# M4THYOU/TokenDagger

Hardware: AMD Instinct MI355X
Metric: GB/s raw text tokenized (Llama-4 vocab, 1024 MB corpus) (higher is better)
Workload: dtype u8; 1 GPU; Llama-4-Scout vocab, 1024 MiB synthetic english text, 1741775 documents, CoreBPE::encode semantics, input resident in HBM; bytes=1073741824, docs=1741775, bytes_rank0=1073741824, docs_rank0=1741775, parallelism=single GPU

## Files before the change

### tokendagger_amd/csrc/td_common.h

```cpp
#pragma once
#include <stdint.h>

#include "../../include/tokendagger_hip.h"

#if defined(__HIP__)
#define TD_HD __host__ __device__ inline __attribute__((always_inline))
#else
#define TD_HD inline
#endif

namespace td {

enum : uint32_t {
    C_OTHER = 0,
    C_APOS = 1,
    C_SLASH = 2,
    C_SP = 3,
    C_WS = 4,
    C_CRLF = 5,
    C_UP = 6,
    C_LW = 7,
    C_LB = 8,
    C_MK = 9,
    C_NUM = 10,
// ... 721 lines not shown
    }
    TD_HD int run_end2(int k1, int k2, int from) const {
        int i = from;
        while (i < lim) {
            const int wi = i >> 6, sh = i & 63;
            const uint64_t m = ((word(k1, wi) | word(k2, wi)) & ~eword(wi)) >> sh;
            const int t = td_ctz64(~m);
            if (t < 64 - sh) return i + t;
            i += 64 - sh;
        }
        return i;
    }
    template <class F>
    TD_HD int last_where(const F& f, int lo, int hi) const {
        if (hi <= lo) return -1;
        for (int wi = (hi - 1) >> 6; wi >= (lo >> 6); --wi) {
            uint64_t m = f(wi);
            const int base = wi << 6;
            if (hi - base < 64) m &= td_bits_below(hi - base);
            if (lo > base) m &= ~td_bits_below(lo - base);
            if (m) return base + td_top64(m) - 1;
        }
        return -1;
    }
    TD_HD int last_and(int k1, int k2, int lo, int hi) const {
        return last_where([&](int wi) { return word(k1, wi) & word(k2, wi); }, lo, hi);
    }
    TD_HD int last_set(int k, int lo, int hi) const {
        return last_where([&](int wi) { return word(k, wi); }, lo, hi);
    }
    TD_HD int last_clear(int k, int lo, int hi) const {
        return last_where([&](int wi) { return ~word(k, wi); }, lo, hi);
    }
};

template <class P, class B>
TD_HD int scan_contraction_p(const P& p, const B& bytes, int e, bool leading = false) {
    if (e + 3 > p.lim) return -1;
    if (!p.bit(MK_A, e) || (p.bit(MK_D, e) && !leading)) return e;
    if (p.bit(MK_D, e + 1)) return e;
    const uint32_t b1 = bytes(e + 1);
    const bool d2 = p.bit(MK_D, e + 2);
    if (b1 < 0x80) {
        const uint32_t l1 = b1 | 0x20;
        if (l1 == 's' || l1 == 't' || l1 == 'm' || l1 == 'd') return e + 2;
        if (d2) return e;
        const uint32_t b2 = bytes(e + 2);
        if (b2 < 0x80) {
            const uint32_t l2 = b2 | 0x20;
            if ((l1 == 'r' && l2 == 'e') || (l1 == 'v' && l2 == 'e') || (l1 == 'l' && l2 == 'l')) return e + 3;
        }
        return e;
    }
    if (b1 == 0xC5 && !d2 && bytes(e + 2) == 0xBF) return e + 3;
    return e;
}

template <class P, class B>
TD_HD int scan_piece_gpt2_p(const P& p, const B& bytes) {
    const int o = p.o, lim = p.lim;
    if (o + 3 > lim) return -1;
    if (p.bit(MK_A, o) && !p.bit(MK_D, o + 1)) {
        const uint32_t b1 = bytes(o + 1);
        if (b1 == 's' || b1 == 't' || b1 == 'm' || b1 == 'd') return o + 2;
        if (!p.bit(MK_D, o + 2)) {
            const uint32_t b2 = bytes(o + 2);
// ... 306 lines not shown
```

### tokendagger_amd/csrc/td_kernels.hip

```cpp
#include <hip/hip_runtime.h>
#include <stdlib.h>

#include "td_kernels.h"

namespace td {

#ifdef TD_ABLATE
#define TD_STOP(n) (a.stop_after == (n))
#else
#define TD_STOP(n) false
#endif

struct LdsSrc {
    const uint8_t* txt;
    const uint32_t* docw;
    int64_t lo, hi;
    __device__ __forceinline__ uint32_t byte(int64_t i) const { return txt[i]; }
    __device__ __forceinline__ bool doc(int64_t i) const { return (docw[i >> 5] >> (i & 31)) & 1u; }
};
struct GlobSrc {
    const uint8_t* text;
    const uint32_t* docbits;
    int64_t lo, hi;
    __device__ __forceinline__ uint32_t byte(int64_t i) const { return text[i]; }
// ... 220 lines not shown
            const bool less = lo + lane < hi && a.doc_offsets[lo + lane] < b0;
            lo += (int64_t)__popcll((unsigned long long)__ballot(less));
        }
        wave_sync_lds();
        for (int64_t d = lo + lane;; d += 64) {
            const int64_t p = d < nd ? a.doc_offsets[d] : b1;
            if (p >= b0 && p < b1 && p < a.n) {
                atomicOr(&bits[(p - b0) >> 5], 1u << (p & 31));
                atomicMin(&first[(p - b0) / K_TILE], (uint32_t)d);
            }
            if (!((__ballot(p < b1 && d < nd) >> 63) & 1ull)) break;
        }
        wave_sync_lds();
#pragma unroll
        for (int q = 0; q < 4; ++q) {
            const int64_t gw = (b0 >> 5) + 4 * (lane + 64 * q);
            if (gw < words) reinterpret_cast<uint4*>(a.docbits)[gw >> 2] = reinterpret_cast<const uint4*>(bits)[lane + 64 * q];
        }
        const int64_t t = b0 / K_TILE + lane;
        if (lane < PM_RANGE / K_TILE && t <= a.n_tiles) a.tile_first_doc[t] = first[lane];
        wave_sync_lds();
    }
}

constexpr int K_MWORDS = K_WIN / 64;

__device__ __forceinline__ uint64_t bits64(const uint32_t* arr, int pos) {
    const int w = pos >> 5, sh = pos & 31;
    const uint64_t lo = ((uint64_t)arr[w + 1] << 32) | arr[w];
    const uint64_t hi = arr[w + 2];
    return sh ? (lo >> sh) | (hi << (64 - sh)) : lo;
}

template <uint32_t PV>
__device__ __noinline__ int scan_piece_lds(const uint64_t* s_mask, const uint8_t* s_txt, int p) {
    const ArrMaskP mp(s_mask, p, K_LIM);
    return scan_piece_p(mp, [s_txt](int q) { return (uint32_t)s_txt[q]; }, PV);
}

__device__ __forceinline__ void load_bitwin(BitWin& w, const uint64_t* s_mask, int base) {
    const int word = base >> 6, sh = base & 63;
    const uint64_t* lo = s_mask + word * MK_COUNT;
    const uint64_t* hi = lo + MK_COUNT;
#pragma unroll
    for (int k = 0; k < MK_COUNT; ++k) w.m[k] = sh ? (lo[k] >> sh) | (hi[k] << (64 - sh)) : lo[k];
}

__device__ __noinline__ uint4 load_text16_edge(const uint8_t* text, int64_t n, int64_t g) {
    uint32_t w[4] = {0, 0, 0, 0};
    for (int k = 0; k < 16; ++k) {
        const int64_t gg = g + k;
        if (gg >= 0 && gg < n) w[k >> 2] |= (uint32_t)text[gg] << ((k & 3) * 8);
    }
    return make_uint4(w[0], w[1], w[2], w[3]);
}
__device__ __forceinline__ uint4 load_text16(const EncodeArgs& a, int64_t g) {
    if (g >= 0 && g + 16 <= a.n && a.text_aligned) return *reinterpret_cast<const uint4*>(a.text + g);
    if (g + 16 > 0 && g < a.n) return load_text16_edge(a.text, a.n, g);
    return make_uint4(0, 0, 0, 0);
}

__device__ __noinline__ uint32_t stage_window_edge(uint8_t* s_txt, const uint8_t* text, int64_t n, int64_t w0, int tid, int n16) {
    uint32_t hib = 0;
    for (int v = tid; v < n16; v += K_THREADS) {
        const int64_t g = w0 + (int64_t)v * 16;
        uint32_t w[4] = {0, 0, 0, 0};
        for (int k = 0; k < 16; ++k) {
            const int64_t gg = g + k;
            if (gg >= 0 && gg < n) w[k >> 2] |= (uint32_t)text[gg] << ((k & 3) * 8);
// ... 242 lines not shown
        int mine = -1;
        const uint32_t o = k + fz_shift_of(meta, pnm, k, &mine);
        if ((v & 0xC0000000u) == TOK_MISS && mine >= 0) {
            const uint32_t nq = meta[mine] >> 16;
            for (uint32_t q = 0; q < nq; ++q) dst[o + q] = (int32_t)mids[mine * 64 + q];
        } else {
            dst[o] = (int32_t)v;
        }
    }
}
__device__ __forceinline__ void fz_stage_with_misses(const uint32_t* slab, uint32_t* st0, uint32_t* mo0, uint32_t pnp, uint32_t pn0, uint32_t pnm) {
    const uint32_t* const meta = slab + SLAB_META;
    const uint32_t* const mids = slab + SLAB_MIDS;
    for (uint32_t k = threadIdx.x; k < pnp; k += K_THREADS) {
        uint32_t v = slab[k];
        if ((v & 0xC0000000u) == TOK_MISS) {
            for (uint32_t q = 0; q < pnm; ++q) {
                const uint32_t e = meta[q];
                if ((e & 0xFFFFu) == k) {
                    const uint32_t mp = meta[SLAB_MAX_MISSES + q], hq = mp >> 12, pos = mp & 0xFFFu, nq = e >> 16;
                    uint32_t* const mo = mo0 + (size_t)hq * K_STAGE + pos;
                    for (uint32_t r = 0; r < nq; ++r) mo[r] = mids[q * 64 + r];
                    v = TOK_MISS | TOK_MERGED | (pos << 7) | nq;
                }
            }
        }
        if (k < pn0) st0[k] = v; else st0[K_STAGE + (k - pn0)] = v;
    }
}

#ifndef TD_SPLIT_MIN_WAVES
#define TD_SPLIT_MIN_WAVES 6
#endif
constexpr int KS_HCAP = 768;
constexpr int KS_CCAP = 128;

constexpr int FZ_NPC = 5120;
#ifndef TD_FZ_PB
#define TD_FZ_PB 1
#endif
constexpr int FZ_PB = TD_FZ_PB;
constexpr int FZ_R_MASK = (K_MWORDS + 1) * MK_COUNT * 8;
constexpr int FZ_R_HEADS = FZ_R_MASK;
constexpr int FZ_R_COLD = FZ_R_HEADS + (KS_HCAP + 2) * 2;
constexpr int FZ_R_SPLIT_END = FZ_R_COLD + KS_CCAP * 2;
constexpr int FZ_R_PLIST = 0;
constexpr int FZ_CCAP = 768;
constexpr int FZ_R_COLDK = ((FZ_NPC + 8) * 2 + 15) & ~15;
constexpr int FZ_R_PB = FZ_R_COLDK + FZ_CCAP * 2;
constexpr int FZ_R_SM = FZ_R_PB + K_THREADS * 2;
constexpr int FZ_R_TOK_END = FZ_R_SM + K_THREADS * 4;
static_assert(SLAB_MIDS >= FZ_NPC + 8, "a slab holds the slots of the fullest tile the fused loop takes");
constexpr int FZ_R_BYTES = ((FZ_R_SPLIT_END > FZ_R_TOK_END ? FZ_R_SPLIT_END : FZ_R_TOK_END) + 15) & ~15;
constexpr int PD_KIND = 0;
constexpr int PD_TILE = 1, PD_NP = 2, PD_N0 = 3, PD_COUNT = 4, PD_NMISS = 5, PD_FDD = 6, PD_EXT0 = 7;
constexpr int PD_WORDS = 8;
static_assert(SLAB_MAX_MISSES == 2 * K_MISS_LISTED_MAX, "slab layout");
#ifndef TD_LB_MAX_POLLS
#define TD_LB_MAX_POLLS 2
#endif
#ifndef TD_LB_DRAIN_POLLS
#define TD_LB_DRAIN_POLLS 64
#endif
#ifndef TD_LB_MAX_ROUNDS
#define TD_LB_MAX_ROUNDS 4
#endif
#ifndef TD_FUSED_MIN_WAVES
#define TD_FUSED_MIN_WAVES 6
#endif

template <uint32_t PV, bool FUSED, bool DIRECT>
__global__ __launch_bounds__(K_THREADS, FUSED ? TD_FUSED_MIN_WAVES : TD_SPLIT_MIN_WAVES) void td_split_tiles(const EncodeArgs a_kern) {
    static_assert(FUSED || !DIRECT, "direct placement is part of the fused tile loop");
    __shared__ __attribute__((aligned(16))) uint8_t s_txt[K_WIN];
    __shared__ __attribute__((aligned(16))) uint8_t s_R[FZ_R_BYTES];
    uint64_t* const s_mask = reinterpret_cast<uint64_t*>(s_R);
    uint16_t* const s_heads = reinterpret_cast<uint16_t*>(s_R + FZ_R_HEADS);
    uint16_t* const s_cold = reinterpret_cast<uint16_t*>(s_R + FZ_R_COLD);
    __shared__ uint32_t s_start[K_WIN / 32 + 3];
    __shared__ uint32_t s_doc[K_WIN / 32 + 2];
    __shared__ uint8_t s_lut[128];
    __shared__ uint8_t s_fcls[16];
    __shared__ uint32_t s_nh, s_cur, s_ncold, s_nonascii;
    __shared__ int s_last;
    __shared__ int s_cross;
    __shared__ uint32_t s_defer;
    __shared__ int s_next[2];

    const int tid = threadIdx.x;
#ifdef TD_FUSED_TIMING
    unsigned long long tt[16] = {0, 0, 0, 0, 0, 0, 0, 0, 0, 0, 0, 0, 0, 0, 0, 0}, t_last = __builtin_readcyclecounter(), t_total0 = t_last, n_tiles_done = 0;
#define FZ_TICK(i) { const unsigned long long t_now = __builtin_readcyclecounter(); tt[i] += t_now - t_last; t_last = t_now; FZ_FRESH }
#else
#define FZ_TICK(i) FZ_FRESH
#endif
#ifndef TD_ARGS_IN_REGISTERS
    (void)a_kern;
    FreshArgs a{kernarg_args()};
    FreshTables T{(const __attribute__((address_space(4))) Tables*)a->Tp};
#define FZ_FRESH { a.refresh(); T.refresh(); }
#else
    const KeptArgs a{&a_kern};
    const Tables T_kept = uniform_tables(a->Tp);
    const KeptTables T{&T_kept};
#define FZ_FRESH
#endif
    for (int q = tid; q < 128; q += K_THREADS) s_lut[q] = (uint8_t)feature_of_class(T->ascii_cls[q]);
    if (tid < 16) s_fcls[tid] = (uint8_t)feature_of_class((uint32_t)tid);
    if (tid == 0) s_nonascii = 0;
    __shared__ __attribute__((aligned(16))) uint32_t s_kmask[FUSED ? (P12_MAXLEN + 1) * 4 : 4];
    __shared__ uint32_t s_wave[8];
    __shared__ uint32_t s_hflags[2], s_nrec[2], s_ncoldp;
    __shared__ uint32_t s_rec[2][K_MISS_LISTED_MAX];
    __shared__ unsigned long long s_pend[48];
    __shared__ uint32_t s_npend;
    __shared__ uint32_t s_flagl[32];
    __shared__ uint32_t s_nflagl;
    __shared__ uint32_t s_pd[DIRECT ? SLAB_RING : 1][PD_WORDS];
    __shared__ uint32_t s_stat[2];
    __shared__ unsigned long long s_lbv[4];
    __shared__ uint32_t s_lbs[4][3];
    __shared__ uint32_t s_brk;
    auto append_pending = [&](uint32_t npd) {
        const int ln = tid & 63;
        const bool have = (uint32_t)ln < npd;
        const unsigned long long rec = have ? s_pend[ln] : 0ull;
        const uint32_t c = mq_class((uint32_t)rec & 127u);
#pragma unroll
        for (uint32_t q = 0; q < (uint32_t)K_MISS_CLASSES; ++q) {
            const uint64_t b = __ballot(have && c == q);
            if (b) {
                const int leader = (int)td_ctz64(b);
                uint32_t at = 0;
                if (ln == leader) at = atomicAdd(&a->miss_count[q], (uint32_t)__popcll((unsigned long long)b));
                at = (uint32_t)__shfl((int)at, leader);
                if (have && c == q) a->miss_list[(size_t)q * a->miss_cap + at + (uint32_t)__popcll((unsigned long long)(b & ((1ull << ln) - 1ull)))] = rec;
            }
        }
    };
    if constexpr (FUSED) {
        if (tid < (int)(P12_MAXLEN + 1) * 4) {
            const int len = tid >> 2, w = tid & 3, nb = len - 4 * w;
// ... 251 lines not shown
                    uint32_t m0 = 0, m1 = 0;
                    for (uint32_t q = 0; q < pnm; ++q) { if (meta[SLAB_MAX_MISSES + q] >> 12) m1 = 1; else m0 = 1; }
                    a->tile_count[tB4] = pn0 | (m0 ? TILE_MISS_LISTED : 0u);
                    a->tile_extra[tB4] = pext0;
                    if (ptwo) {
                        a->tile_count[tB4 + 1] = (pnp - pn0) | (m1 ? TILE_MISS_LISTED : 0u);
                        a->tile_extra[tB4 + 1] = pcount - pnp - pext0;
                    }
                    if (base == -1) {
                        __hip_atomic_store(&a->tile_state[B], TS_BROKEN << 62, __ATOMIC_RELAXED, __HIP_MEMORY_SCOPE_AGENT);
                        s_brk = 1u;
                    } else {
                        s_stat[1] += 1u;
                    }
                }
            }
            if (tid == 0) s_pd[ring][PD_KIND] = 0;
            FZ_TICK(11)
        }
        if (!have) {
            __syncthreads();
            ring = __builtin_amdgcn_readfirstlane(ring + 1 == SLAB_RING ? 0 : ring + 1);
            continue;
        }
        {
        FZ_TICK(0)
        const bool tile_ascii = !s_nonascii;

        LdsSrc src;
        src.txt = s_txt;
        src.docw = s_doc;
        src.lo = (wg0 < 0) ? -wg0 : 0;
        src.hi = (a->n - wg0 < K_WIN) ? (a->n - wg0) : K_WIN;
        if (tid < MK_COUNT) s_mask[K_MWORDS * MK_COUNT + tid] = 0;
        auto emit_masks = [&](int it, uint32_t flo, uint32_t fhi, uint32_t pf) {
            const uint64_t P = transpose8x8(((uint64_t)fhi << 32) | flo);
            const uint32_t plo = (uint32_t)P, phi = (uint32_t)(P >> 32);
            const uint32_t mU = plo & 0xFF, mW = (plo >> 8) & 0xFF, mX = (plo >> 16) & 0xFF, mS = plo >> 24;
            const uint32_t nraw = phi & 0xFF, mCR = (phi >> 8) & 0xFF, mSL = (phi >> 16) & 0xFF, mC = phi >> 24;
            const uint32_t mN = nraw & ~mX & ~mS, mA = nraw & mX, mSP = nraw & mS;
            const uint32_t mD = reinterpret_cast<const uint8_t*>(s_doc)[it];
            const uint32_t mSY = sync_byte(mU, mW, mX, mS, mN, mCR, mSL, mC, mD, mA, pf, PV);
            static_assert(MK_U == 0 && MK_W == 1 && MK_X == 2 && MK_S == 3 && MK_N == 4 && MK_CR == 5 && MK_TR == 6 &&
                          MK_C == 7 && MK_D == 8 && MK_A == 9 && MK_SP == 10 && MK_SYNC == 11, "mask order");
            uint8_t* o = reinterpret_cast<uint8_t*>(s_mask + (it >> 3) * MK_COUNT) + (it & 7);
            o[0 * 8] = (uint8_t)mU; o[1 * 8] = (uint8_t)mW; o[2 * 8] = (uint8_t)mX; o[3 * 8] = (uint8_t)mS;
            o[4 * 8] = (uint8_t)mN; o[5 * 8] = (uint8_t)mCR; o[6 * 8] = (uint8_t)(mCR | mSL); o[7 * 8] = (uint8_t)mC;
            o[8 * 8] = (uint8_t)mD; o[9 * 8] = (uint8_t)mA; o[10 * 8] = (uint8_t)mSP; o[11 * 8] = (uint8_t)mSY;
        };
        constexpr int P1_ITEMS = K_WIN / 8;
        if (tile_ascii) {
            for (int it = tid; it < P1_ITEMS; it += K_THREADS) {
                const uint2 t8 = reinterpret_cast<const uint2*>(s_txt)[it];
                const uint32_t flo = (uint32_t)s_lut[t8.x & 0x7F] | ((uint32_t)s_lut[(t8.x >> 8) & 0x7F] << 8) |
                                     ((uint32_t)s_lut[(t8.x >> 16) & 0x7F] << 16) | ((uint32_t)s_lut[t8.x >> 24] << 24);
                const uint32_t fhi = (uint32_t)s_lut[t8.y & 0x7F] | ((uint32_t)s_lut[(t8.y >> 8) & 0x7F] << 8) |
                                     ((uint32_t)s_lut[(t8.y >> 16) & 0x7F] << 16) | ((uint32_t)s_lut[t8.y >> 24] << 24);
                uint32_t pf = __shfl_up(fhi >> 24, 1);
                if (lane == 0) pf = it > 0 ? (uint32_t)s_lut[s_txt[it * 8 - 1]] : 0u;
                emit_masks(it, flo, fhi, pf);
            }
        } else {
        constexpr int P1_WAVES = K_THREADS / 64, P1_PER_WAVE = (P1_ITEMS / P1_WAVES) & ~63;
        static_assert(P1_ITEMS - P1_WAVES * P1_PER_WAVE <= 64, "the items left over are one more pass of the last wavefront");
        uint32_t carry_st = 0x100u, carry_pf = 0;
        const int n_pass = P1_PER_WAVE / 64 + ((tid >> 6) == P1_WAVES - 1 ? 1 : 0);
        const uint8_t* const t_ascii = T->ascii_cls;
        const uint16_t* const t_u1 = T->ucls1;
        const uint8_t* const t_u2 = T->ucls2;
        for (int q = 0; q < n_pass; ++q) {
            const int it = (tid >> 6) * P1_PER_WAVE + q * 64 + lane;
            if (it >= P1_ITEMS) break;
            const uint2 t8 = reinterpret_cast<const uint2*>(s_txt)[it];
            uint32_t flo, fhi;
            uint32_t st_out = 0;
            int lead_conts = 0;
            if (!((t8.x | t8.y) & 0x80808080u)) {
                flo = (uint32_t)s_lut[t8.x & 0x7F] | ((uint32_t)s_lut[(t8.x >> 8) & 0x7F] << 8) |
                      ((uint32_t)s_lut[(t8.x >> 16) & 0x7F] << 16) | ((uint32_t)s_lut[t8.x >> 24] << 24);
                fhi = (uint32_t)s_lut[t8.y & 0x7F] | ((uint32_t)s_lut[(t8.y >> 8) & 0x7F] << 8) |
                      ((uint32_t)s_lut[(t8.y >> 16) & 0x7F] << 16) | ((uint32_t)s_lut[t8.y >> 24] << 24);
// ... 91 lines not shown
            {
                uint32_t st_in = __shfl_up(st_out, 1);
                if (lane == 0) st_in = carry_st;
                carry_st = (uint32_t)__builtin_amdgcn_readlane((int)st_out, 63);
                if (lead_conts) {
                    const bool known = !(st_in & 0x100u);
                    const int claim = (int)(st_in >> 9);
                    for (int k = 0; k < lead_conts; ++k) {
                        const uint32_t f = (known && k < claim) ? ((st_in & 0xFFu) | FB_C) : feature_at_v(t_ascii, t_u1, t_u2, s_txt, s_doc, (int)src.lo, (int)src.hi, it * 8 + k);
                        if (k < 4) flo |= f << (8 * k); else fhi |= f << (8 * (k - 4));
                    }
                }
            }
            uint32_t pf = __shfl_up(fhi >> 24, 1);
            if (lane == 0 && q > 0) pf = carry_pf;
            carry_pf = (uint32_t)__builtin_amdgcn_readlane((int)(fhi >> 24), 63);
            if (lane == 0 && q == 0) {
                pf = 0;
                if (it > 0) {
                    const uint32_t pb = s_txt[it * 8 - 1];
                    pf = (pb < 0x80) ? (uint32_t)s_lut[pb] : feature_at_v(t_ascii, t_u1, t_u2, s_txt, s_doc, (int)src.lo, (int)src.hi, it * 8 - 1);
                }
            }
            emit_masks(it, flo, fhi, pf);
        }
        }
        __syncthreads();
        FZ_TICK(1)
        if (tid == 0) s_nonascii = 0;
        if (TD_STOP(12)) continue;

        {
            constexpr bool FAST = !(PV & (PV_GPT2 | PV_LEADING_CONTRACTION | PV_PLAIN_LETTERS | PV_WS_EOS_FIRST));
            const uint32_t* s_mask32 = reinterpret_cast<const uint32_t*>(s_mask);
            auto dword_at = [](int j) { return (j >> 1) * (MK_COUNT * 2) + (j & 1); };
            auto defer = [&](int64_t g) {
                if (FUSED) s_defer = 1;
                const uint32_t q = atomicAdd(a->slow_count, 1u);
                if (q < a->slow_cap) a->slow_list[q] = g;
                else raise(a, TD_E_SCRATCH, g);
            };
            auto mark = [&](int q) { atomicOr(&s_start[q >> 5], 1u << (q & 31)); };
            auto sync_at = [&](int q) { return (s_mask32[dword_at(q >> 5) + 2 * MK_SYNC] >> (q & 31)) & 1u; };
            auto crossed = [&](int e) {
                if (FUSED) s_cross = e;
                if (tile + 1 < a->n_stiles) a->tile_carry[tile + 1] = wg0 + e;
            };
            auto walk = [&](int p) {
                for (;;) {
                    const int e = scan_piece_lds<PV>(s_mask, s_txt, p);
                    if (e < 0) { if (p >= K_HL) defer(wg0 + p); return; }
                    if (e >= tile_hi) { crossed(e); return; }
                    if (sync_at(e)) return;
                    if (e >= K_HL) mark(e);
                    p = e;
                }
            };
            const int b0 = K_HL + tid * 32;
            uint32_t mine = 0;
            uint32_t extra_hi = 0;
            {
                const uint32_t* lo = s_mask32 + dword_at(b0 >> 5);
                const uint32_t* hi = s_mask32 + dword_at((b0 >> 5) + 1);
                BitWin wv;
#pragma unroll
                for (int k = 0; k < MK_COUNT; ++k) wv.m[k] = ((uint64_t)hi[2 * k] << 32) | lo[2 * k];
                uint32_t sy = (uint32_t)wv.m[MK_SYNC];
                const int room = tile_hi - b0;
                if (room < 32) sy = room <= 0 ? 0u : sy & ((1u << room) - 1u);
                uint32_t st0 = sy, un;
                if (wv.m[MK_N] != 0ull) {
                    uint64_t extra = 0;
                    un = (uint32_t)split_unresolved_heads(wv, PV, &extra) & sy;
                    extra &= (uint64_t)sy << 3;
                    extra &= room >= 64 ? ~0ull : room <= 0 ? 0ull : ((1ull << room) - 1ull);
                    st0 |= (uint32_t)extra;
                    extra_hi = (uint32_t)(extra >> 32);
                } else {
                    un = (uint32_t)split_unresolved_heads(wv, PV) & sy;
                }
                s_start[b0 >> 5] = st0;
                if (sy) atomicMax(&s_last, b0 + 31 - (int)__clz(sy));
                const uint32_t cnt = __popc(un);
                const uint32_t incl = wave_incl_scan(cnt, lane);
                uint32_t base = 0;
                if (lane == 63 && incl) base = atomicAdd(&s_nh, incl);
                base = (uint32_t)__builtin_amdgcn_readlane((int)base, 63);
                uint32_t idx = base + incl - cnt;
                while (un) {
                    const int bit = __ffs(un) - 1;
                    un &= un - 1u;
                    if (idx < (uint32_t)KS_HCAP) s_heads[idx] = (uint16_t)(b0 + bit); else mine |= 1u << bit;
                    ++idx;
                }
            }
            __syncthreads();
            FZ_TICK(2)
            if (extra_hi) atomicOr(&s_start[(b0 >> 5) + 1], extra_hi);
            if (TD_STOP(13)) continue;
            {
                const uint32_t nh = s_nh < (uint32_t)KS_HCAP ? s_nh : (uint32_t)KS_HCAP;
                int p = -1;
                if (tid == 0) {
                    static_assert(K_HL % 64 == 0 && K_HL >= 64, "left halo = whole mask words");
                    if (!(s_mask[(K_HL / 64) * MK_COUNT + MK_SYNC] & 1ull)) {
                        int sp = -1;
                        for (int w = K_HL / 64 - 1; w >= 0 && sp < 0; --w) {
                            uint64_t m = s_mask[w * MK_COUNT + MK_SYNC];
                            if (w == 0) m &= ~0xFull;
                            if (m) sp = w * 64 + td_top64(m) - 1;
                        }
                        if (sp < 0) { a->tile_flag[tile] = 1; atomicAdd(a->far_count, 1u); if (FUSED) s_defer = 1; }
                        else p = sp;
                    }
                }
                if (tid == 1 && s_last >= 0) p = s_last;
                bool more = true;
                for (;;) {
                    const uint64_t nb = __ballot(p < 0);
                    if (nb && more) {
                        uint32_t base = 0;
                        if (lane == __ffsll((unsigned long long)nb) - 1) base = atomicAdd(&s_cur, (uint32_t)__popcll(nb));
                        base = (uint32_t)__builtin_amdgcn_readlane((int)base, __ffsll((unsigned long long)nb) - 1);
                        more = base + (uint32_t)__popcll(nb) < nh;
                        if (p < 0) {
                            const uint32_t idx = base + __builtin_amdgcn_mbcnt_hi((uint32_t)(nb >> 32), __builtin_amdgcn_mbcnt_lo((uint32_t)nb, 0u));
                            if (idx < nh) p = s_heads[idx];
                        }
                    }
                    if (!__ballot(p >= 0)) break;
                    if (p >= 0) {
                        const int sh = p & 31;
                        const uint32_t* lo = s_mask32 + dword_at(p >> 5);
                        const uint32_t* hi = s_mask32 + dword_at((p >> 5) + 1);
                        BitWin32 v;
#pragma unroll
                        for (int k = 0; k < MK_COUNT; ++k) v.m[k] = __funnelshift_r(lo[2 * k], hi[2 * k], (uint32_t)sh);
                        const int avail = (K_LIM - p < 32) ? (K_LIM - p) : 32;
                        auto bytes = [&](int q) { return (uint32_t)s_txt[p + q]; };
                        const int r = FAST ? scan_piece_fast32(v, avail, bytes, PV) : scan_piece_p(WinP32(v, avail), bytes, PV);
                        if (r < 0) {
                            const uint32_t ci = atomicAdd(&s_ncold, 1u);
                            if (ci < (uint32_t)KS_CCAP) s_cold[ci] = (uint16_t)p; else walk(p);
                            p = -1;
                        } else {
                            const int e = p + r;
                            bool stop = true;
                            if (e >= tile_hi) crossed(e);
                            else {
                                stop = (r < 32) ? ((v.m[MK_SYNC] >> r) & 1u) : sync_at(e);
                                if (!stop && e >= K_HL) mark(e);
                            }
                            p = stop ? -1 : e;
                        }
                    }
                }
            }
            __syncthreads();
            {
                const uint32_t nc = s_ncold < (uint32_t)KS_CCAP ? s_ncold : (uint32_t)KS_CCAP;
                for (uint32_t i = tid; i < nc; i += K_THREADS) walk(s_cold[i]);
                while (mine) {
                    const int bit = __ffs(mine) - 1;
                    mine &= mine - 1u;
                    walk(b0 + bit);
                }
            }
        }
        __syncthreads();
        FZ_TICK(3)
        if (tid < KS_TILE / 32) {
            const int64_t g = tile_g0 + (int64_t)tid * 32;
            if (g < a->n) {
                uint32_t v = s_start[K_HL / 32 + tid];
                if (g + 32 > a->n) v &= (1u << (int)(a->n - g)) - 1u;
                TD_NT_STORE(v, &a->startbits[(tile_g0 >> 5) + tid]);
            }
        }
        if constexpr (DRAW) {
            if constexpr (!DIRECT) {
                next_tile = __builtin_amdgcn_readfirstlane(s_next[par]);
                if (tid == 0) s_next[par ^ 1] = (int)(2u * gridDim.x + atomicAdd(a->tile_draw, 1u));
                par = __builtin_amdgcn_readfirstlane(par ^ 1);
            } else {
                next_tile = __builtin_amdgcn_readfirstlane(s_next[0]);
            }
            if (next_tile < a->n_stiles) load_window((int64_t)next_tile * KS_TILE - K_HL);
        } else if (FUSED && tile + (int)gridDim.x < a->n_stiles) {
            load_window(wg0 + (int64_t)gridDim.x * KS_TILE);
        }
        }
        if constexpr (FUSED) {
            constexpr int NT4 = KS_TILE / K_TILE;
            static_assert(NT4 == 2 && KS_CHUNK == 32, "two token tiles, a 32-bit START word per lane");
            const int cross = s_cross;
            const bool tile_deferred = s_defer != 0 || cross < 0;
            uint16_t* const s_plist = reinterpret_cast<uint16_t*>(s_R + FZ_R_PLIST);
            uint16_t* const s_coldk = reinterpret_cast<uint16_t*>(s_R + FZ_R_COLDK);
            uint16_t* const s_pb = reinterpret_cast<uint16_t*>(s_R + FZ_R_PB);
            uint32_t* const s_sm = reinterpret_cast<uint32_t*>(s_R + FZ_R_SM);
            const int wv = tid >> 6;
            const int tile4 = tile * NT4;
            const bool two = K_HL + K_TILE < tile_hi;
            const int b0 = K_HL + tid * KS_CHUNK;
            const uint32_t smask0 = s_start[b0 >> 5];
            const uint32_t cnt = __popc(smask0);
            const uint32_t incl = wave_incl_scan(cnt, lane);
            if (lane == 63) s_wave[wv] = incl;
            if (tid == 0) { s_hflags[0] = 0; s_hflags[1] = 0; s_nrec[0] = 0; s_nrec[1] = 0; s_ncoldp = 0; }
            __syncthreads();
            const uint32_t w0s = s_wave[0], w1s = s_wave[1], w2s = s_wave[2], w3s = s_wave[3];
            const uint32_t np = w0s + w1s + w2s + w3s, n0 = w0s + w1s;
            const uint32_t pbase = (wv > 0 ? w0s : 0u) + (wv > 1 ? w1s : 0u) + (wv > 2 ? w2s : 0u) + incl - cnt;
            const bool cand = DIRECT && !s_brk;
            auto break_chain = [&]() {
                __hip_atomic_store(&a->tile_state[tile], TS_BROKEN << 62, __ATOMIC_RELAXED, __HIP_MEMORY_SCOPE_AGENT);
                s_brk = 1u;
            };
            if (tile_deferred || np > (uint32_t)FZ_NPC) {
                if (tid == 0) {
                    const uint32_t at = atomicAdd(a->deferred_count, two ? 2u : 1u);
                    a->deferred_list[at] = (uint32_t)tile4;
                    if (two) a->deferred_list[at + 1] = (uint32_t)tile4 + 1u;
                    if (DIRECT) break_chain();
                }
            } else {
                {
                    uint32_t k = pbase, m = smask0;
                    while (m) {
                        const int b = __ffs(m) - 1;
                        m &= m - 1;
                        s_plist[k++] = (uint16_t)(b0 + b);
                    }
                }
                s_pb[tid] = (uint16_t)pbase;
                s_sm[tid] = smask0;
                if (tid == 0) s_plist[np] = (uint16_t)cross;
                const uint64_t fdd = fd0 != 0xFFFFFFFFu ? fd0 : fd1;
                if (cand && tid == 0) { s_pd[ring][PD_FDD] = (uint32_t)fdd; s_pd[ring][PD_TILE] = (uint32_t)tile; s_pd[ring][PD_NP] = np; s_pd[ring][PD_N0] = n0; }
                const int64_t dmine = (int64_t)fdd + tid;
                const int64_t dpos = (fdd != 0xFFFFFFFFu && dmine < a->n_docs) ? a->doc_offsets[dmine] : a->n;
                __syncthreads();
                FZ_TICK(4)
                uint32_t* const slab = a->slab + ((size_t)blockIdx.x * SLAB_RING + ring) * SLAB_WORDS;
                uint32_t* const dst0 = cand ? slab : a->stage + (size_t)tile4 * K_STAGE;
                uint32_t* const dst1 = cand ? slab : dst0 + K_STAGE - n0;
                auto note_miss = [&](uint32_t k, uint32_t res) {
                    const uint32_t h = k >= n0 ? 1u : 0u;
                    const uint32_t mi = atomicAdd(&s_nrec[h], 1u);
                    if (mi < (uint32_t)K_MISS_LISTED_MAX) s_rec[h][mi] = ((k - (h ? n0 : 0u)) << 19) | (res & 0x7FFFFu);
                };
                auto miss_marker = [&](int i, uint32_t len) { return TOK_MISS | ((uint32_t)((i - K_HL) & (K_TILE - 1)) << 7) | len; };
                typedef uint32_t u32x4 __attribute__((ext_vector_type(4)));
                typedef const u32x4 __attribute__((address_space(1)))* gslot_t;
                gslot_t const p12 = (gslot_t)(uintptr_t)T->piece12_slots;
                const uint32_t p12_mask = T->piece12_mask;
                const bool fastpath = a->use_fastpath != 0;
                for (uint32_t kb = tid; kb < np; kb += K_THREADS * FZ_PB) {
                    u32x4 sl[FZ_PB];
                    uint32_t kk0[FZ_PB], kk1[FZ_PB], kk2[FZ_PB], il[FZ_PB];
#pragma unroll
                    for (int q = 0; q < FZ_PB; ++q) {
                        const uint32_t k = kb + (uint32_t)q * K_THREADS;
                        const bool on = k < np;
                        const int i = on ? s_plist[k] : K_HL;
                        const uint32_t len = on ? (uint32_t)s_plist[k + 1] - (uint32_t)i : 0u;
                        const uint32_t* wp = reinterpret_cast<const uint32_t*>(s_txt) + (i >> 2);
                        const uint32_t sh = (i & 3) * 8;
                        const uint32_t w0 = wp[0], w1 = wp[1], w2 = wp[2], w3 = wp[3];
// ... 52 lines not shown
                        a->deferred_list[at] = (uint32_t)tile4;
                        if (two) a->deferred_list[at + 1] = (uint32_t)tile4 + 1u;
                        if (DIRECT) break_chain();
                    }
                } else if (resolved) {
                    FZ_TICK(12)
                    if (tid < 64) {
                        const uint32_t nr0 = s_nrec[0], nr1 = s_nrec[1], nm = nr0 + nr1;
                        uint32_t ext0 = 0, ext1 = 0;
                        if (nm) {
                            static_assert(2 * SLAB_MAX_MISSES * 4 * MG_UNIT * 4 <= FZ_R_COLDK, "keys + ids of the merged pieces fit the (dead) piece list");
                            uint32_t rec = 0, hh = 0;
                            if ((uint32_t)lane < nm) {
                                hh = (uint32_t)lane >= nr0 ? 1u : 0u;
                                rec = s_rec[hh][(uint32_t)lane - (hh ? nr0 : 0u)];
                            }
                            const uint32_t nt = fz_merge_piece(a->Tp, a->text, a->n, reinterpret_cast<uint32_t*>(s_R), slab, rec, hh, n0, tile_g0, a->err, a->err_pos);
                            const uint32_t e0 = wave_incl_scan((nt && !hh) ? nt - 1u : 0u, lane), e1 = wave_incl_scan((nt && hh) ? nt - 1u : 0u, lane);
                            ext0 = (uint32_t)__builtin_amdgcn_readlane((int)e0, 63);
                            ext1 = (uint32_t)__builtin_amdgcn_readlane((int)e1, 63);
                        }
                        FZ_TICK(13)
                        if (tid == 0) {
                            const uint32_t count = s_pd[ring][PD_NP] + ext0 + ext1;
                            s_pd[ring][PD_KIND] = 1u; s_pd[ring][PD_COUNT] = count; s_pd[ring][PD_NMISS] = nm; s_pd[ring][PD_EXT0] = ext0;
                            __hip_atomic_store(&a->tile_state[s_pd[ring][PD_TILE]], (TS_AGG << 62) | (unsigned long long)count, __ATOMIC_RELAXED, __HIP_MEMORY_SCOPE_AGENT);
                        }
                    }
                    FZ_TICK(7)
                    {
                        const int64_t tile_end_g = wg0 + tile_hi;
                        auto slot_of = [&](int64_t p) {
                            const int lp = (int)(p - tile_g0);
                            const uint32_t k = (uint32_t)s_pb[lp >> 5] + __popc(s_sm[lp >> 5] & ((1u << (lp & 31)) - 1u));
                            return k >= n0 ? k - n0 : k;
                        };
                        if (dpos < tile_end_g) {
                            a->doc_slot[dmine] = slot_of(dpos);
                            for (int64_t d = dmine + K_THREADS; d < a->n_docs; d += K_THREADS) {
                                const int64_t p = a->doc_offsets[d];
                                if (p >= tile_end_g) break;
                                a->doc_slot[d] = slot_of(p);
                            }
                        }
                    }
                    FZ_TICK(9)
                } else {
                if (DIRECT && tid == 0) {
                    break_chain();
                    if (cand) { s_pd[ring][PD_KIND] = 2u; s_pd[ring][PD_NMISS] = 0; }
                }
                if (tid < 64) {
#pragma unroll
                    for (uint32_t h = 0; h < 2; ++h) {
                        const uint32_t nr = s_nrec[h], np0 = s_npend;
                        const bool listed = nr && nr <= (uint32_t)K_MISS_LISTED_MAX;
                        if (listed && (uint32_t)tid < nr) s_pend[np0 + tid] = ((unsigned long long)((uint32_t)tile4 + h) << 32) | s_rec[h][tid];
                        const uint32_t np1 = listed ? np0 + nr : np0;
                        wave_sync_lds();
                        if (np1 > 48u - (uint32_t)K_MISS_LISTED_MAX) {
                            append_pending(np1);
                            wave_sync_lds();
                            if (tid == 0) s_npend = 0;
                        } else if (tid == 0) {
                            s_npend = np1;
                        }
                        wave_sync_lds();
                    }
                    if (tid == 0) {
#pragma unroll
                        for (uint32_t h = 0; h < 2; ++h) {
                            if (h == 1 && !two) break;
                            uint32_t fl = s_hflags[h];
                            const uint32_t nr = s_nrec[h];
                            if (nr > (uint32_t)K_MISS_LISTED_MAX) {
                                fl |= TILE_HAS_MISS;
                                uint32_t nf = s_nflagl;
                                s_flagl[nf++] = (uint32_t)tile4 + h;
                                if (nf == 32u) {
                                    const uint32_t at = atomicAdd(a->flagged_count, 32u);
                                    for (uint32_t q = 0; q < 32u; ++q) a->flagged_list[at + q] = s_flagl[q];
                                    nf = 0;
                                }
                                s_nflagl = nf;
                            } else if (nr) {
                                fl |= TILE_MISS_LISTED;
                            }
                            a->tile_count[tile4 + h] = (h ? np - n0 : n0) | fl;
                        }
                    }
                }
                FZ_TICK(7)
                {
                    const int64_t tile_end_g = wg0 + tile_hi;
                    auto slot_of = [&](int64_t p) {
                        const int lp = (int)(p - tile_g0);
                        const uint32_t k = (uint32_t)s_pb[lp >> 5] + __popc(s_sm[lp >> 5] & ((1u << (lp & 31)) - 1u));
                        return k >= n0 ? k - n0 : k;
                    };
                    if (dpos < tile_end_g) {
                        a->doc_slot[dmine] = slot_of(dpos);
                        for (int64_t d = dmine + K_THREADS; d < a->n_docs; d += K_THREADS) {
                            const int64_t p = a->doc_offsets[d];
                            if (p >= tile_end_g) break;
                            a->doc_slot[d] = slot_of(p);
                        }
                    }
                }
                FZ_TICK(9)
                }
            }
        }
        __syncthreads();
        ring = __builtin_amdgcn_readfirstlane(ring + 1 == SLAB_RING ? 0 : ring + 1);
        FZ_TICK(10)
#ifdef TD_FUSED_TIMING
        ++n_tiles_done;
#endif
    }
#ifdef TD_FUSED_TIMING
    if (FUSED && tid == 0 && (blockIdx.x % 211) == 0)
        printf("fused wg %d: %llu tiles, total %llu cycles | stage %llu masks %llu rules %llu heads %llu | list %llu probe %llu cold %llu bookkeeping %llu lookback %llu docs %llu tail %llu place %llu | t12 %llu t13 %llu\n",
               (int)blockIdx.x, n_tiles_done, (unsigned long long)(__builtin_readcyclecounter() - t_total0), tt[0], tt[1], tt[2], tt[3], tt[4], tt[5], tt[6], tt[7],
               tt[8], tt[9], tt[10], tt[11], tt[12], tt[13]);
#endif
    if constexpr (FUSED) {
        if (DIRECT && tid == 0 && s_stat[0]) atomicAdd(a->direct_tiles, s_stat[0]);
        if (DIRECT && tid == 0 && s_stat[1]) atomicAdd(a->direct_tiles + 1, s_stat[1]);
        if (tid < 64) append_pending(s_npend);
        if (tid == 0 && s_nflagl) {
// ... 3599 lines not shown
```

Measured before the change: 465.7 GB/s.

## Compact LDS mask storage to nine planes and raise fused-kernel occupancy to seven

Stores only nine of the twelve per-byte mask planes in LDS, in a planar 32-bit layout. The doc, apostrophe and space-prefix planes are now derived on read from the raw and doc bits. It also drops the s_sm array, reusing s_start bits for slot lookup, and shrinks the head, cold and piece capacities so the fused kernel fits seven workgroups per CU instead of six. This trades extra ALU work on every mask read, plus smaller per-tile capacity limits that may push more tiles onto slow paths, for higher occupancy.

```diff
diff --git a/tokendagger_amd/csrc/td_common.h b/tokendagger_amd/csrc/td_common.h
--- a/tokendagger_amd/csrc/td_common.h
+++ b/tokendagger_amd/csrc/td_common.h
@@ -777,6 +777,80 @@
     TD_HD int last_clear(int k, int lo, int hi) const {
         return last_where([&](int wi) { return ~word(k, wi); }, lo, hi);
     }
+};
+
+enum : int { CM_U = 0, CM_W, CM_X, CM_S, CM_NRAW, CM_CR, CM_TR, CM_C, CM_SYNC, CM_COUNT };
+template <class V, class W>
+TD_HD void cm_expand(V& v, const W* s, W d) {
+    v.m[MK_U] = s[CM_U]; v.m[MK_W] = s[CM_W]; v.m[MK_X] = s[CM_X]; v.m[MK_S] = s[CM_S];
+    v.m[MK_N] = s[CM_NRAW] & ~(s[CM_X] | s[CM_S]);
+    v.m[MK_CR] = s[CM_CR]; v.m[MK_TR] = s[CM_TR]; v.m[MK_C] = s[CM_C];
+    v.m[MK_D] = d;
+    v.m[MK_A] = s[CM_NRAW] & s[CM_X];
+    v.m[MK_SP] = s[CM_NRAW] & s[CM_S];
+    v.m[MK_SYNC] = s[CM_SYNC];
+}
+struct CompactMaskP {
+    const uint32_t* arr;
+    const uint32_t* doc;
+    int stride;
+    int o, lim;
+    TD_HD CompactMaskP(const uint32_t* a, int stride_, const uint32_t* d, int o_, int lim_) : arr(a), doc(d), stride(stride_), o(o_), lim(lim_) {}
+    TD_HD uint64_t stored(int s, int wi) const { return ((uint64_t)arr[s * stride + 2 * wi + 1] << 32) | arr[s * stride + 2 * wi]; }
+    TD_HD uint64_t dword64(int wi) const { return ((uint64_t)doc[2 * wi + 1] << 32) | doc[2 * wi]; }
+    TD_HD uint64_t word(int k, int wi) const {
+        switch (k) {
+            case MK_U: return stored(CM_U, wi);
+            case MK_W: return stored(CM_W, wi);
+            case MK_X: return stored(CM_X, wi);
+            case MK_S: return stored(CM_S, wi);
+            case MK_N: return stored(CM_NRAW, wi) & ~(stored(CM_X, wi) | stored(CM_S, wi));
+            case MK_CR: return stored(CM_CR, wi);
+            case MK_TR: return stored(CM_TR, wi);
+            case MK_C: return stored(CM_C, wi);
+            case MK_D: return dword64(wi);
+            case MK_A: return stored(CM_NRAW, wi) & stored(CM_X, wi);
+            case MK_SP: return stored(CM_NRAW, wi) & stored(CM_S, wi);
+            default: return stored(CM_SYNC, wi);
+        }
+    }
+    TD_HD uint64_t eword(int wi) const {
+        const int wo = o >> 6;
+        if (wi < wo) return 0;
+        const uint64_t d = dword64(wi);
+        return wi == wo ? d & ~td_bits_below((o & 63) + 1) : d;
+    }
+    TD_HD bool bit(int k, int i) const { return (word(k, i >> 6) >> (i & 63)) & 1ull; }
+    TD_HD bool ebit(int i) const { return i > o && bit(MK_D, i); }
+    template <class F>
+    TD_HD int run_where(const F& f, int from) const {
+        int i = from;
+        while (i < lim) {
+            const int wi = i >> 6, sh = i & 63;
+            const uint64_t m = (f(wi) & ~eword(wi)) >> sh;
+            const int t = td_ctz64(~m);
+            if (t < 64 - sh) return i + t;
+            i += 64 - sh;
+        }
+        return i;
+    }
+    TD_HD int run_end(int k, int from) const { return run_where([&](int wi) { return word(k, wi); }, from); }
+    TD_HD int run_end2(int k1, int k2, int from) const { return run_where([&](int wi) { return word(k1, wi) | word(k2, wi); }, from); }
+    template <class F>
+    TD_HD int last_where(const F& f, int lo, int hi) const {
+        if (hi <= lo) return -1;
+        for (int wi = (hi - 1) >> 6; wi >= (lo >> 6); --wi) {
+            uint64_t m = f(wi);
+            const int base = wi << 6;
+            if (hi - base < 64) m &= td_bits_below(hi - base);
+            if (lo > base) m &= ~td_bits_below(lo - base);
+            if (m) return base + td_top64(m) - 1;
+        }
+        return -1;
+    }
+    TD_HD int last_and(int k1, int k2, int lo, int hi) const { return last_where([&](int wi) { return word(k1, wi) & word(k2, wi); }, lo, hi); }
+    TD_HD int last_set(int k, int lo, int hi) const { return last_where([&](int wi) { return word(k, wi); }, lo, hi); }
+    TD_HD int last_clear(int k, int lo, int hi) const { return last_where([&](int wi) { return ~word(k, wi); }, lo, hi); }
 };
 
 template <class P, class B>
diff --git a/tokendagger_amd/csrc/td_kernels.hip b/tokendagger_amd/csrc/td_kernels.hip
--- a/tokendagger_amd/csrc/td_kernels.hip
+++ b/tokendagger_amd/csrc/td_kernels.hip
@@ -276,9 +276,10 @@
     return sh ? (lo >> sh) | (hi << (64 - sh)) : lo;
 }
 
+constexpr int CM_STRIDE = (K_MWORDS + 1) * 2;
 template <uint32_t PV>
-__device__ __noinline__ int scan_piece_lds(const uint64_t* s_mask, const uint8_t* s_txt, int p) {
-    const ArrMaskP mp(s_mask, p, K_LIM);
+__device__ __noinline__ int scan_piece_lds(const uint32_t* s_cm, const uint32_t* s_doc, const uint8_t* s_txt, int p) {
+    const CompactMaskP mp(s_cm, CM_STRIDE, s_doc, p, K_LIM);
     return scan_piece_p(mp, [s_txt](int q) { return (uint32_t)s_txt[q]; }, PV);
 }
 
@@ -587,24 +588,23 @@
 #ifndef TD_SPLIT_MIN_WAVES
 #define TD_SPLIT_MIN_WAVES 6
 #endif
-constexpr int KS_HCAP = 768;
+constexpr int KS_HCAP = 576;
 constexpr int KS_CCAP = 128;
 
-constexpr int FZ_NPC = 5120;
+constexpr int FZ_NPC = 4736;
 #ifndef TD_FZ_PB
 #define TD_FZ_PB 1
 #endif
 constexpr int FZ_PB = TD_FZ_PB;
-constexpr int FZ_R_MASK = (K_MWORDS + 1) * MK_COUNT * 8;
+constexpr int FZ_R_MASK = CM_STRIDE * CM_COUNT * 4;
 constexpr int FZ_R_HEADS = FZ_R_MASK;
 constexpr int FZ_R_COLD = FZ_R_HEADS + (KS_HCAP + 2) * 2;
 constexpr int FZ_R_SPLIT_END = FZ_R_COLD + KS_CCAP * 2;
 constexpr int FZ_R_PLIST = 0;
-constexpr int FZ_CCAP = 768;
+constexpr int FZ_CCAP = 512;
 constexpr int FZ_R_COLDK = ((FZ_NPC + 8) * 2 + 15) & ~15;
 constexpr int FZ_R_PB = FZ_R_COLDK + FZ_CCAP * 2;
-constexpr int FZ_R_SM = FZ_R_PB + K_THREADS * 2;
-constexpr int FZ_R_TOK_END = FZ_R_SM + K_THREADS * 4;
+constexpr int FZ_R_TOK_END = FZ_R_PB + K_THREADS * 2;
 static_assert(SLAB_MIDS >= FZ_NPC + 8, "a slab holds the slots of the fullest tile the fused loop takes");
 constexpr int FZ_R_BYTES = ((FZ_R_SPLIT_END > FZ_R_TOK_END ? FZ_R_SPLIT_END : FZ_R_TOK_END) + 15) & ~15;
 constexpr int PD_KIND = 0;
@@ -621,15 +621,19 @@
 #define TD_LB_MAX_ROUNDS 4
 #endif
 #ifndef TD_FUSED_MIN_WAVES
-#define TD_FUSED_MIN_WAVES 6
+#define TD_FUSED_MIN_WAVES 7
 #endif
 
+#ifndef TD_DIRECT_MIN_WAVES
+#define TD_DIRECT_MIN_WAVES 6
+#endif
+static_assert(TD_FUSED_MIN_WAVES < 7 || FZ_R_BYTES <= 11072, "seven workgroups per CU: 22 752 B of LDS each, of which s_R may have 11 072");
 template <uint32_t PV, bool FUSED, bool DIRECT>
-__global__ __launch_bounds__(K_THREADS, FUSED ? TD_FUSED_MIN_WAVES : TD_SPLIT_MIN_WAVES) void td_split_tiles(const EncodeArgs a_kern) {
+__global__ __launch_bounds__(K_THREADS, !FUSED ? TD_SPLIT_MIN_WAVES : DIRECT ? TD_DIRECT_MIN_WAVES : TD_FUSED_MIN_WAVES) void td_split_tiles(const EncodeArgs a_kern) {
     static_assert(FUSED || !DIRECT, "direct placement is part of the fused tile loop");
     __shared__ __attribute__((aligned(16))) uint8_t s_txt[K_WIN];
     __shared__ __attribute__((aligned(16))) uint8_t s_R[FZ_R_BYTES];
-    uint64_t* const s_mask = reinterpret_cast<uint64_t*>(s_R);
+    uint32_t* const s_cm = reinterpret_cast<uint32_t*>(s_R);
     uint16_t* const s_heads = reinterpret_cast<uint16_t*>(s_R + FZ_R_HEADS);
     uint16_t* const s_cold = reinterpret_cast<uint16_t*>(s_R + FZ_R_COLD);
     __shared__ uint32_t s_start[K_WIN / 32 + 3];
@@ -663,6 +667,8 @@
     for (int q = tid; q < 128; q += K_THREADS) s_lut[q] = (uint8_t)feature_of_class(T->ascii_cls[q]);
     if (tid < 16) s_fcls[tid] = (uint8_t)feature_of_class((uint32_t)tid);
     if (tid == 0) s_nonascii = 0;
+    if (tid < 2) s_doc[K_WIN / 32 + tid] = 0;
+    static_assert(K_WIN / 32 + 2 == CM_STRIDE, "the document bits cover the words the stored masks have");
     __shared__ __attribute__((aligned(16))) uint32_t s_kmask[FUSED ? (P12_MAXLEN + 1) * 4 : 4];
     __shared__ uint32_t s_wave[8];
     __shared__ uint32_t s_hflags[2], s_nrec[2], s_ncoldp;
@@ -980,21 +986,22 @@
         src.docw = s_doc;
         src.lo = (wg0 < 0) ? -wg0 : 0;
         src.hi = (a->n - wg0 < K_WIN) ? (a->n - wg0) : K_WIN;
-        if (tid < MK_COUNT) s_mask[K_MWORDS * MK_COUNT + tid] = 0;
+        if (tid < 2 * CM_COUNT) s_cm[(tid >> 1) * CM_STRIDE + 2 * K_MWORDS + (tid & 1)] = 0;
         auto emit_masks = [&](int it, uint32_t flo, uint32_t fhi, uint32_t pf) {
             const uint64_t P = transpose8x8(((uint64_t)fhi << 32) | flo);
             const uint32_t plo = (uint32_t)P, phi = (uint32_t)(P >> 32);
             const uint32_t mU = plo & 0xFF, mW = (plo >> 8) & 0xFF, mX = (plo >> 16) & 0xFF, mS = plo >> 24;
             const uint32_t nraw = phi & 0xFF, mCR = (phi >> 8) & 0xFF, mSL = (phi >> 16) & 0xFF, mC = phi >> 24;
-            const uint32_t mN = nraw & ~mX & ~mS, mA = nraw & mX, mSP = nraw & mS;
+            const uint32_t mN = nraw & ~mX & ~mS, mA = nraw & mX;
             const uint32_t mD = reinterpret_cast<const uint8_t*>(s_doc)[it];
             const uint32_t mSY = sync_byte(mU, mW, mX, mS, mN, mCR, mSL, mC, mD, mA, pf, PV);
-            static_assert(MK_U == 0 && MK_W == 1 && MK_X == 2 && MK_S == 3 && MK_N == 4 && MK_CR == 5 && MK_TR == 6 &&
-                          MK_C == 7 && MK_D == 8 && MK_A == 9 && MK_SP == 10 && MK_SYNC == 11, "mask order");
-            uint8_t* o = reinterpret_cast<uint8_t*>(s_mask + (it >> 3) * MK_COUNT) + (it & 7);
-            o[0 * 8] = (uint8_t)mU; o[1 * 8] = (uint8_t)mW; o[2 * 8] = (uint8_t)mX; o[3 * 8] = (uint8_t)mS;
-            o[4 * 8] = (uint8_t)mN; o[5 * 8] = (uint8_t)mCR; o[6 * 8] = (uint8_t)(mCR | mSL); o[7 * 8] = (uint8_t)mC;
-            o[8 * 8] = (uint8_t)mD; o[9 * 8] = (uint8_t)mA; o[10 * 8] = (uint8_t)mSP; o[11 * 8] = (uint8_t)mSY;
+            static_assert(CM_U == 0 && CM_W == 1 && CM_X == 2 && CM_S == 3 && CM_NRAW == 4 && CM_CR == 5 && CM_TR == 6 &&
+                          CM_C == 7 && CM_SYNC == 8, "stored mask order");
+            uint8_t* o = reinterpret_cast<uint8_t*>(s_cm) + it;
+            constexpr int MB = CM_STRIDE * 4;
+            o[0 * MB] = (uint8_t)mU; o[1 * MB] = (uint8_t)mW; o[2 * MB] = (uint8_t)mX; o[3 * MB] = (uint8_t)mS;
+            o[4 * MB] = (uint8_t)nraw; o[5 * MB] = (uint8_t)mCR; o[6 * MB] = (uint8_t)(mCR | mSL); o[7 * MB] = (uint8_t)mC;
+            o[8 * MB] = (uint8_t)mSY;
         };
         constexpr int P1_ITEMS = K_WIN / 8;
         if (tile_ascii) {
@@ -1152,8 +1159,18 @@
 
         {
             constexpr bool FAST = !(PV & (PV_GPT2 | PV_LEADING_CONTRACTION | PV_PLAIN_LETTERS | PV_WS_EOS_FIRST));
-            const uint32_t* s_mask32 = reinterpret_cast<const uint32_t*>(s_mask);
-            auto dword_at = [](int j) { return (j >> 1) * (MK_COUNT * 2) + (j & 1); };
+            auto load_view64 = [&](BitWin& v, int j) {
+                uint64_t s[CM_COUNT];
+#pragma unroll
+                for (int k = 0; k < CM_COUNT; ++k) s[k] = ((uint64_t)s_cm[k * CM_STRIDE + j + 1] << 32) | s_cm[k * CM_STRIDE + j];
+                cm_expand(v, s, ((uint64_t)s_doc[j + 1] << 32) | s_doc[j]);
+            };
+            auto load_view32 = [&](BitWin32& v, int j, uint32_t sh) {
+                uint32_t s[CM_COUNT];
+#pragma unroll
+                for (int k = 0; k < CM_COUNT; ++k) s[k] = __funnelshift_r(s_cm[k * CM_STRIDE + j], s_cm[k * CM_STRIDE + j + 1], sh);
+                cm_expand(v, s, __funnelshift_r(s_doc[j], s_doc[j + 1], sh));
+            };
             auto defer = [&](int64_t g) {
                 if (FUSED) s_defer = 1;
                 const uint32_t q = atomicAdd(a->slow_count, 1u);
@@ -1161,14 +1178,14 @@
                 else raise(a, TD_E_SCRATCH, g);
             };
             auto mark = [&](int q) { atomicOr(&s_start[q >> 5], 1u << (q & 31)); };
-            auto sync_at = [&](int q) { return (s_mask32[dword_at(q >> 5) + 2 * MK_SYNC] >> (q & 31)) & 1u; };
+            auto sync_at = [&](int q) { return (s_cm[CM_SYNC * CM_STRIDE + (q >> 5)] >> (q & 31)) & 1u; };
             auto crossed = [&](int e) {
                 if (FUSED) s_cross = e;
                 if (tile + 1 < a->n_stiles) a->tile_carry[tile + 1] = wg0 + e;
             };
             auto walk = [&](int p) {
                 for (;;) {
-                    const int e = scan_piece_lds<PV>(s_mask, s_txt, p);
+                    const int e = scan_piece_lds<PV>(s_cm, s_doc, s_txt, p);
                     if (e < 0) { if (p >= K_HL) defer(wg0 + p); return; }
                     if (e >= tile_hi) { crossed(e); return; }
                     if (sync_at(e)) return;
@@ -1180,11 +1197,8 @@
             uint32_t mine = 0;
             uint32_t extra_hi = 0;
             {
-                const uint32_t* lo = s_mask32 + dword_at(b0 >> 5);
-                const uint32_t* hi = s_mask32 + dword_at((b0 >> 5) + 1);
                 BitWin wv;
-#pragma unroll
-                for (int k = 0; k < MK_COUNT; ++k) wv.m[k] = ((uint64_t)hi[2 * k] << 32) | lo[2 * k];
+                load_view64(wv, b0 >> 5);
                 uint32_t sy = (uint32_t)wv.m[MK_SYNC];
                 const int room = tile_hi - b0;
                 if (room < 32) sy = room <= 0 ? 0u : sy & ((1u << room) - 1u);
@@ -1223,10 +1237,11 @@
                 int p = -1;
                 if (tid == 0) {
                     static_assert(K_HL % 64 == 0 && K_HL >= 64, "left halo = whole mask words");
-                    if (!(s_mask[(K_HL / 64) * MK_COUNT + MK_SYNC] & 1ull)) {
+                    const uint32_t* const sync32 = s_cm + CM_SYNC * CM_STRIDE;
+                    if (!(sync32[K_HL / 32] & 1u)) {
                         int sp = -1;
                         for (int w = K_HL / 64 - 1; w >= 0 && sp < 0; --w) {
-                            uint64_t m = s_mask[w * MK_COUNT + MK_SYNC];
+                            uint64_t m = ((uint64_t)sync32[2 * w + 1] << 32) | sync32[2 * w];
                             if (w == 0) m &= ~0xFull;
                             if (m) sp = w * 64 + td_top64(m) - 1;
                         }
@@ -1250,12 +1265,8 @@
                     }
                     if (!__ballot(p >= 0)) break;
                     if (p >= 0) {
-                        const int sh = p & 31;
-                        const uint32_t* lo = s_mask32 + dword_at(p >> 5);
-                        const uint32_t* hi = s_mask32 + dword_at((p >> 5) + 1);
                         BitWin32 v;
-#pragma unroll
-                        for (int k = 0; k < MK_COUNT; ++k) v.m[k] = __funnelshift_r(lo[2 * k], hi[2 * k], (uint32_t)sh);
+                        load_view32(v, p >> 5, (uint32_t)(p & 31));
                         const int avail = (K_LIM - p < 32) ? (K_LIM - p) : 32;
                         auto bytes = [&](int q) { return (uint32_t)s_txt[p + q]; };
                         const int r = FAST ? scan_piece_fast32(v, avail, bytes, PV) : scan_piece_p(WinP32(v, avail), bytes, PV);
@@ -1318,7 +1329,6 @@
             uint16_t* const s_plist = reinterpret_cast<uint16_t*>(s_R + FZ_R_PLIST);
             uint16_t* const s_coldk = reinterpret_cast<uint16_t*>(s_R + FZ_R_COLDK);
             uint16_t* const s_pb = reinterpret_cast<uint16_t*>(s_R + FZ_R_PB);
-            uint32_t* const s_sm = reinterpret_cast<uint32_t*>(s_R + FZ_R_SM);
             const int wv = tid >> 6;
             const int tile4 = tile * NT4;
             const bool two = K_HL + K_TILE < tile_hi;
@@ -1354,7 +1364,6 @@
                     }
                 }
                 s_pb[tid] = (uint16_t)pbase;
-                s_sm[tid] = smask0;
                 if (tid == 0) s_plist[np] = (uint16_t)cross;
                 const uint64_t fdd = fd0 != 0xFFFFFFFFu ? fd0 : fd1;
                 if (cand && tid == 0) { s_pd[ring][PD_FDD] = (uint32_t)fdd; s_pd[ring][PD_TILE] = (uint32_t)tile; s_pd[ring][PD_NP] = np; s_pd[ring][PD_N0] = n0; }
@@ -1473,7 +1482,7 @@
                         const int64_t tile_end_g = wg0 + tile_hi;
                         auto slot_of = [&](int64_t p) {
                             const int lp = (int)(p - tile_g0);
-                            const uint32_t k = (uint32_t)s_pb[lp >> 5] + __popc(s_sm[lp >> 5] & ((1u << (lp & 31)) - 1u));
+                            const uint32_t k = (uint32_t)s_pb[lp >> 5] + __popc(s_start[K_HL / 32 + (lp >> 5)] & ((1u << (lp & 31)) - 1u));
                             return k >= n0 ? k - n0 : k;
                         };
                         if (dpos < tile_end_g) {
@@ -1536,7 +1545,7 @@
                     const int64_t tile_end_g = wg0 + tile_hi;
                     auto slot_of = [&](int64_t p) {
                         const int lp = (int)(p - tile_g0);
-                        const uint32_t k = (uint32_t)s_pb[lp >> 5] + __popc(s_sm[lp >> 5] & ((1u << (lp & 31)) - 1u));
+                        const uint32_t k = (uint32_t)s_pb[lp >> 5] + __popc(s_start[K_HL / 32 + (lp >> 5)] & ((1u << (lp & 31)) - 1u));
                         return k >= n0 ? k - n0 : k;
                     };
                     if (dpos < tile_end_g) {
```

New measurement: 491.7 GB/s, median of 6. +5.6%, better.
